# Bazs/structure_from_motion

Measured on NVIDIA B200. Metric: hyp x point evals/sec (fp64), higher is better.
Workload: dtype f64

## Files before the change

### structure_from_motion_b200/csrc/sfm_api.cu

```cuda
#include "../../include/sfm_b200.h"

#include <dlfcn.h>

#include <cmath>
#include <cstdarg>
#include <cstdio>
#include <cstdlib>
#include <cstring>
#include <string>
#include <vector>

#include "sfm_device.cuh"
#include "sfm_fit.cuh"
#include "sfm_linalg.cuh"
#include "sfm_score.cuh"
#include "sfm_homography.cuh"
#include "sfm_pose.cuh"
#include "sfm_tail.cuh"
#include "sfm_misc.cuh"
#include "sfm_match.cuh"
#include "sfm_harris.cuh"
#include "sfm_select.cuh"

using namespace sfm;

static_assert(sizeof(Corr) == 32, "Corr must be 32 bytes");
static_assert(sizeof(PoseSet) == sizeof(sfm_poses), "PoseSet/sfm_poses layout mismatch");
static_assert(sizeof(SelectRecord) == SFM_RECORD_BYTES, "SelectRecord / SFM_RECORD_BYTES mismatch");
static_assert(sizeof(ModelScores) == sizeof(sfm_model_scores), "ModelScores / sfm_model_scores layout mismatch");

namespace {

thread_local std::string g_err;
// ... 43 lines not shown
    T* as() const { return reinterpret_cast<T*>(p); }
    void release() {
        if (p) cudaFree(p);
        p = nullptr;
        cap = 0;
    }
};

enum { T_UPLOAD = 0, T_SAMPLE, T_FIT, T_SCORE, T_SELECT, T_MASK, T_POSE, T_TRI, T_COUNT };

}

struct sfm_ctx {
    int device = 0;
    int sm_count = 148;
    cudaStream_t own_stream = nullptr, stream = nullptr;
    Buf raw, pts, offsets, Ks, table, E, valid, eig;
    Buf acc, count_extra, S1, S2, err, blocks, best, invalid, winnerE, spts, bounds, fitflag, record, merged, rows, blockinv;
    Buf m_img, m_feat, m_W, m_ss, m_ok, m_S, m_out;
    Buf h_img, h_gx, h_gy, h_corner, h_alive, h_key, h_idx, h_small, h_xy;
    Buf mask, sed, poses, pass, X, idx, scan, tmp, tailstate, num, winrec, bout;
    Buf planes, hK;
    Buf selstate, selio, selpp;
    long long n = 0, h = 0, npairs = 1;
    long long first_len = 0;
    long long batch_max_len = 0;
    long long raw_stride = 1;
    bool batched = false, has_pts = false, has_table = false, has_models = false, has_score = false;
    bool models_h = false;
    int hscore_occ = 0;
    bool table_pending = false;
    unsigned long long smp_seed = 0, smp_stream = 0;
    long long smp_offset = 0;
    bool acc_clean = false;
    size_t acc_planes_for = 0;
    double Kstage[9] = {0};
    double hstage[18] = {0};
    std::vector<SelectModels> sstage;
    std::vector<double> Kbatch;
    const void* occ_fn[4] = {nullptr, nullptr, nullptr, nullptr};
    int occ_blocks[4] = {0, 0, 0, 0};
    int occ_next = 0;
    void* nccl_comm = nullptr;
    int nccl_rank = 0, nccl_world = 1;
    Buf gathered;
    const unsigned long long* rescored_dev = nullptr;
    long long winner_local = -1;
    bool winner_set = false;
    long long last_idx_offset = 0;
    double Khost[9] = {1, 0, 0, 0, 1, 0, 0, 0, 1};
    int variant = SFM_SCORE_AUTO, hpt = 2, group = 16;
    bool timing = false;
    cudaEvent_t ev0[T_COUNT], ev1[T_COUNT];
    bool ev_used[T_COUNT];
    long long launches = 0;
    void* hpin = nullptr;
    size_t hpin_cap = 0;

    void tic(int s) {
        if (timing) { cudaEventRecord(ev0[s], stream); }
    }
    void toc(int s) {
        if (timing) { cudaEventRecord(ev1[s], stream); ev_used[s] = true; }
    }
// ... 49 lines not shown
    cfg->attrs = at;
    cfg->numAttrs = SFM_PDL ? 1 : 0;
}
template <typename... KArgs, typename... Args>
cudaError_t chain_launch(sfm_ctx* c, void (*kernel)(KArgs...), dim3 grid, dim3 block, size_t smem, Args&&... args) {
    cudaLaunchConfig_t cfg;
    cudaLaunchAttribute at;
    chain_config(c, grid, block, smem, &cfg, &at);
    return cudaLaunchKernelEx(&cfg, kernel, static_cast<KArgs>(args)...);
}
inline cudaError_t chain_launch_ptr(sfm_ctx* c, const void* fn, dim3 grid, dim3 block, size_t smem, void** kargs) {
    cudaLaunchConfig_t cfg;
    cudaLaunchAttribute at;
    chain_config(c, grid, block, smem, &cfg, &at);
    return cudaLaunchKernelExC(&cfg, fn, kargs);
}

size_t score_warp_smem(int hpt, bool full) {
    switch (hpt) {
        case 1: return full ? score_warp_bytes<1, MODE_FULL>() : sizeof(ScoreWarpSmem<1>);
        case 2: return full ? score_warp_bytes<2, MODE_FULL>() : sizeof(ScoreWarpSmem<2>);
        case 4: return full ? score_warp_bytes<4, MODE_FULL>() : sizeof(ScoreWarpSmem<4>);
        default: return sizeof(ScoreWarpSmem<8>);
    }
}

const void* score_kernel(int variant, int hpt, int group) {
    if (variant == SFM_SCORE_SCREEN32) {
#define SFM_K32(H, G) if (hpt == H && group == G) return reinterpret_cast<const void*>(&k_score<H, G, MODE_SCREEN32>)
        SFM_K32(2, 16); SFM_K32(4, 8); SFM_K32(8, 4);
#undef SFM_K32
        return nullptr;
    }
#define SFM_K(H, G) if (hpt == H && group == G) return scr ? reinterpret_cast<const void*>(&k_score<H, G, MODE_SCREEN>) \
                                                           : reinterpret_cast<const void*>(&k_score<H, G, MODE_FULL>)
    const bool scr = variant == SFM_SCORE_SCREEN;
    SFM_K(1, 16); SFM_K(1, 32);
    SFM_K(2, 4); SFM_K(2, 8); SFM_K(2, 16);
    SFM_K(4, 2); SFM_K(4, 4); SFM_K(4, 8);
#undef SFM_K
    return nullptr;
}

}

extern "C" {
// ... 227 lines not shown
    c->npairs = 1;
    const double* s[4];
    if (on_device) {
        if (int r = c->raw.reserve((size_t)n * 4 * sizeof(double))) return r;
        double* d = c->raw.as<double>();
        const double* src[4] = {xa, ya, xb, yb};
        for (int k = 0; k < 4; ++k) {
            CU(cudaMemcpy2DAsync(d + (size_t)k * n, sizeof(double), src[k], (size_t)stride * sizeof(double),
                                 sizeof(double), (size_t)n, cudaMemcpyDeviceToDevice, c->stream));
            s[k] = d + (size_t)k * n;
        }
        c->raw_stride = stride = 1;
    } else if (int r = stage_raw(c, xa, ya, xb, yb, stride, n, s)) {
        return r;
    }
    if (int r = c->Ks.reserve(9 * sizeof(double))) return r;
    memcpy(c->Khost, K, sizeof c->Khost);
    CU(cudaMemcpyAsync(c->Ks.p, c->Khost, 9 * sizeof(double), cudaMemcpyHostToDevice, c->stream));
    c->n = n;
    if (int r = normalise_from(c, s[0], s[1], s[2], s[3], stride, n, n)) return r;
    c->toc(T_UPLOAD);
    if (sync) CU(cudaStreamSynchronize(c->stream));
    c->has_pts = true;
    c->has_table = c->has_models = c->has_score = false;
    c->table_pending = false;
    c->winner_set = false;
    return 0;
}

int sfm_upload_pairs(sfm_ctx* c, const double* xa, const double* ya, const double* xb, const double* yb,
                     int64_t stride, int64_t n, const double* K) {
    return upload_pairs_impl(c, xa, ya, xb, yb, stride, n, K, false, true);
}

int sfm_upload_pairs_async(sfm_ctx* c, const double* xa, const double* ya, const double* xb, const double* yb,
                           int64_t stride, int64_t n, const double* K) {
    return upload_pairs_impl(c, xa, ya, xb, yb, stride, n, K, false, false);
}

int sfm_upload_pairs_d(sfm_ctx* c, const double* xa, const double* ya, const double* xb, const double* yb,
                       int64_t stride, int64_t n, const double* K) {
    return upload_pairs_impl(c, xa, ya, xb, yb, stride, n, K, true, true);
}

int sfm_get_normalised(sfm_ctx* c, double* out, int64_t n) {
    if (int r = use(c)) return r;
// ... 98 lines not shown
    if (int r = c->S1.reserve(H * 8)) return r;
    if (int r = c->S2.reserve(H * 8)) return r;
    if (int r = c->err.reserve(H * 8)) return r;
    if (int r = c->blocks.reserve((size_t)fblocks * P * sizeof(Best))) return r;
    if (int r = c->best.reserve((size_t)P * sizeof(Best))) return r;
    if (int r = c->invalid.reserve((size_t)P * 16)) return r;
    return 0;
}

struct ItemSplit { long long chunk, nsplit; };
static ItemSplit split_items(long long target_items, long long hyp_items, long long max_len, long long tile) {
    const long long tiles = (max_len + tile - 1) / tile;
    long long nsplit = (target_items + hyp_items - 1) / hyp_items;
    constexpr int min_tiles = 2;
    const long long max_split = tiles / min_tiles > 0 ? tiles / min_tiles : 1;
    if (nsplit > max_split) nsplit = max_split;
    const long long min_split = (max_len + kMaxItemPoints - 1) / kMaxItemPoints;
    if (nsplit < min_split) nsplit = min_split;
    if (nsplit < 1) nsplit = 1;
    const long long chunk = ((tiles + nsplit - 1) / nsplit) * tile;
    nsplit = (max_len + chunk - 1) / chunk;
    if (nsplit < 1) nsplit = 1;
    return {chunk, nsplit};
}

static int clear_acc(sfm_ctx* c, size_t H, long long P) {
    if (!(c->acc_clean && c->acc_planes_for == H))
        CU(cudaMemsetAsync(c->acc.p, 0, H * kAccWords * 8 + acc_tail_bytes(P), c->stream));
    c->acc_clean = false;
    return 0;
}

static int finalise_launch(sfm_ctx* c, int kind, double thr, double min_extra, int agg, int mode, bool use_table,
                           long long idx_offset, int sums, int e2, int force_rescore, unsigned long long* acc_dev) {
    const long long h = c->h, P = c->npairs;
    const size_t H = (size_t)h * P;
    const int fblocks = (int)((h + 255) / 256);
    c->tic(T_SELECT);
    FinalArgs f;
    f.pts = c->pts.as<Corr>();
    f.offsets = c->batched ? c->offsets.as<long long>() : nullptr;
    f.E = c->E.as<double>();
    f.valid = c->valid.as<uint8_t>();
    f.table = use_table ? c->table.as<int32_t>() : nullptr;
    f.h = h;
    f.n = c->n;
// ... 51 lines not shown
    const int G = (c->variant == SFM_SCORE_SCREEN32 && thr > 1e6) ? 16 : c->group;
    const long long hblocks = (h + 32ll * hpt - 1) / (32ll * hpt);
    const size_t H = (size_t)h * P;
    if (int r = reserve_selection(c, h, P)) return r;
    int e2 = 0;
    if (thr > 0.0 && !skip_k2) (void)frexp(thr, &e2);
    if (e2 < -400) e2 = -400;
    const bool autov = c->variant == SFM_SCORE_AUTO;
    int variant = autov ? SFM_SCORE_SCREEN : c->variant;
    if (variant == SFM_SCORE_SCREEN32 && thr > 1e6) variant = SFM_SCORE_SCREEN;
    const bool f32 = variant == SFM_SCORE_SCREEN32;
    const bool screen = variant != SFM_SCORE_FULL;
    double thr_pre = f32 ? thr * kThr32Factor : (screen ? thr * (1.0 + 1e-9) : thr * (1.0 + 1e-9) + 1e-22);
    if (f32 && thr_pre < 1e-24) thr_pre = 1e-24;
    if (screen && thr_pre < 1e-280) thr_pre = 1e-280;
    const double s_scale = sqrt(thr_pre);
    const double scale1 = ldexp(1.0, 63 - e2), scale2 = ldexp(1.0, 63 - 2 * e2);
    unsigned long long* acc_dev = nullptr;
    {
        const void* fn = score_kernel(variant, hpt, G);
        if (!fn) return fail(SFM_ERR_ARG, "unsupported scoring configuration (variant %d, hpt %d, group %d)", variant, hpt, G);
        const size_t smem_one = (size_t)kScoreWarps * score_warp_smem(hpt, false);
        const size_t smem_two = (size_t)kScoreWarps * score_warp_smem(hpt, true);
        const size_t smem_both = smem_one > smem_two ? smem_one : smem_two;
        const size_t smem = screen ? smem_one : smem_two;
        auto occupancy = [&](const void* f, size_t bytes, int* out) -> int {
            for (int k = 0; k < 4; ++k)
                if (c->occ_fn[k] == f) { *out = c->occ_blocks[k]; return 0; }
            int o = 0;
            CU(cudaFuncSetAttribute(f, cudaFuncAttributeMaxDynamicSharedMemorySize, (int)bytes));
            CU(cudaOccupancyMaxActiveBlocksPerMultiprocessor(&o, f, kScoreThreads, bytes));
            if (o < 1) o = 1;
            c->occ_fn[c->occ_next] = f;
            c->occ_blocks[c->occ_next] = o;
            c->occ_next = (c->occ_next + 1) & 3;
            *out = o;
            return 0;
        };
        int occ = 0;
        if (int r = occupancy(fn, smem, &occ)) return r;
#ifndef SFM_AUTO_SINGLE
#define SFM_AUTO_SINGLE 1
#endif
        const void* fn_auto = nullptr;
        if (autov && SFM_AUTO_SINGLE) {
            if (hpt == 2 && G == 16) fn_auto = reinterpret_cast<const void*>(&k_score_auto<2, 16>);
            if (hpt == 4 && G == 8) fn_auto = reinterpret_cast<const void*>(&k_score_auto<4, 8>);
        }
        if (fn_auto)
            if (int r = occupancy(fn_auto, smem_both, &occ)) return r;
        const void* fn_full = (autov && !fn_auto) ? score_kernel(SFM_SCORE_FULL, hpt, G) : nullptr;
        int occ_full = 0;
        if (fn_full)
            if (int r = occupancy(fn_full, smem_two, &occ_full)) return r;
        const long long grid_blocks = (long long)c->sm_count * occ;
        constexpr int items_per_warp = 32;
        const ItemSplit sp = split_items(grid_blocks * kScoreWarps * items_per_warp, hblocks * P, max_len, kTile);
        const long long chunk = sp.chunk, nsplit = sp.nsplit;
        const long long total_items = hblocks * nsplit * P;
        if (int r = c->acc.reserve(H * kAccWords * 8 + acc_tail_bytes(P))) return r;
        const long long npts = c->n;
        if (f32) { if (int r = c->spts.reserve((size_t)npts * sizeof(Corr32))) return r; }
        else if (screen) { if (int r = c->spts.reserve((size_t)npts * sizeof(Corr))) return r; }
        ScoreArgs a;
        a.pts = c->pts.as<Corr>();
        a.spts = screen ? c->spts.p : c->pts.p;
        a.bounds = c->bounds.as<double>();
        a.s = s_scale;
        a.kappa_coef = kKappaCoef * (1.0 + thr);
        a.kappa32_coef = kKappa32Coef * (1.0 + thr);
        a.n = c->n;
        a.offsets = c->batched ? c->offsets.as<long long>() : nullptr;
        a.E = c->E.as<double>();
        a.rows = c->rows.as<ModelRow>();
        a.h = h;
        a.thr = thr;
        a.thr_pre = thr_pre;
        a.scale1 = scale1;
        a.scale2 = scale2;
        a.sums = sums;
        a.chunk = chunk;
        a.hblocks = (int)hblocks;
        a.nsplit = (int)nsplit;
        a.total_items = total_items;
        a.htotal = (long long)H;
        a.acc = c->acc.as<unsigned long long>();
        a.work_counter = reinterpret_cast<unsigned*>(a.acc + H * kAccWords);
        char* tailp = reinterpret_cast<char*>(a.acc + H * kAccWords);
        a.mode_flag = autov ? reinterpret_cast<const int*>(tailp + 32) : nullptr;
        acc_dev = a.acc;
        c->tic(T_SCORE);
        if (int r = clear_acc(c, H, P)) return r;
        if (f32 && !skip_k2) {
            k_screen_pts32<<<(unsigned)((npts + 255) / 256), 256, 0, c->stream>>>(c->pts.as<Corr>(), npts, 1.0 / s_scale,
                                                                                  reinterpret_cast<Corr32*>(c->spts.p));
            if (int r = check_launch(c, "k_screen_pts32")) return r;
        }
        else if (screen && !skip_k2) {
            PilotArgs pa;
            pa.E = c->E.as<double>();
            pa.h = h;
            pa.plen = c->batched ? c->first_len : c->n;
            pa.thr_pre = thr_pre;
            pa.counters = reinterpret_cast<unsigned*>(tailp + 16);
            pa.mode_flag = autov ? reinterpret_cast<int*>(tailp + 32) : nullptr;
            CU(chain_launch(c, k_screen_pts64, dim3((unsigned)((npts + 255) / 256)), dim3(256), 0, c->pts.as<Corr>(), npts,
                            1.0 / s_scale, reinterpret_cast<Corr*>(c->spts.p), pa));
            if (int r = check_launch(c, "k_screen_pts64")) return r;
        }
        const long long want_blocks = (total_items + kScoreWarps - 1) / kScoreWarps;
        const long long launch_blocks = grid_blocks < want_blocks ? grid_blocks : want_blocks;
        void* kargs[] = {(void*)&a};
        if (!skip_k2 && fn_auto) {
            ScoreArgs a2 = a;
            a2.thr_pre = thr * (1.0 + 1e-9) + 1e-22;
            a2.spts = c->pts.p;
            void* kargs2[] = {(void*)&a, (void*)&a2};
            CU(chain_launch_ptr(c, fn_auto, dim3((unsigned)launch_blocks), dim3(kScoreThreads), smem_both, kargs2));
            if (int r = check_launch(c, "k_score_auto")) return r;
        } else if (!skip_k2) {
            CU(chain_launch_ptr(c, fn, dim3((unsigned)launch_blocks), dim3(kScoreThreads), smem, kargs));
            if (int r = check_launch(c, "k_score")) return r;
            if (fn_full) {
                ScoreArgs a2 = a;
                a2.thr_pre = thr * (1.0 + 1e-9) + 1e-22;
                a2.spts = c->pts.p;
                const long long gb2 = (long long)c->sm_count * occ_full;
                const long long lb2 = gb2 < want_blocks ? gb2 : want_blocks;
                void* kargs2[] = {(void*)&a2};
                CU(chain_launch_ptr(c, fn_full, dim3((unsigned)lb2), dim3(kScoreThreads), smem_two, kargs2));
                if (int r = check_launch(c, "k_score")) return r;
            }
        }
        c->toc(T_SCORE);
    }

    return finalise_launch(c, MODEL_E, thr, min_extra, agg, mode, use_table, idx_offset, sums, e2, force_rescore, acc_dev);
}

int sfm_score(sfm_ctx* c, double thr, double min_extra, int agg, int mode, int use_table, int64_t idx_offset,
              int32_t* count_extra, double* S1, double* S2, double* err) {
    if (int r = use(c)) return r;
    if (c->batched) return fail(SFM_ERR_STATE, "sfm_score is a single-pair call; use sfm_batch_ransac");
    if (int r = score_launch(c, thr, min_extra, agg, mode, use_table != 0, idx_offset, c->n, S1 || S2)) return r;
    const size_t H = (size_t)c->h;
    if (count_extra) CU(cudaMemcpyAsync(count_extra, c->count_extra.p, H * 4, cudaMemcpyDeviceToHost, c->stream));
    if (S1) CU(cudaMemcpyAsync(S1, c->S1.p, H * 8, cudaMemcpyDeviceToHost, c->stream));
    if (S2) CU(cudaMemcpyAsync(S2, c->S2.p, H * 8, cudaMemcpyDeviceToHost, c->stream));
// ... 892 lines not shown
    c->npairs = npairs;
    c->n = n;
    c->first_len = offsets[1] - offsets[0];
    if (int r = c->offsets.reserve((size_t)(npairs + 1) * 8)) return r;
    if (int r = c->Ks.reserve((size_t)npairs * 72)) return r;
    CU(cudaMemcpyAsync(c->offsets.p, offsets, (size_t)(npairs + 1) * 8, cudaMemcpyHostToDevice, c->stream));
    CU(cudaMemcpyAsync(c->Ks.p, Ks, (size_t)npairs * 72, cudaMemcpyHostToDevice, c->stream));
    c->Kbatch.assign(Ks, Ks + 9 * npairs);
    c->batch_max_len = max_len;
    const double* s[4];
    if (int r = stage_raw(c, xa, ya, xb, yb, stride, n, s)) return r;
    if (pixels) {
        const double I[9] = {1, 0, 0, 0, 1, 0, 0, 0, 1};
        if (int r = hpose_stage_k(c, I)) return r;
        if (int r = c->pts.reserve((size_t)n * sizeof(Corr))) return r;
        k_normalise<<<dim3((unsigned)((n + 255) / 256), 1), 256, 0, c->stream>>>(s[0], s[1], s[2], s[3], stride, n, nullptr,
                                                                                c->hK.as<double>(), c->pts.as<Corr>(), nullptr);
        if (int r = check_launch(c, "k_normalise")) return r;
    } else if (int r = normalise_from(c, s[0], s[1], s[2], s[3], stride, n, max_len)) {
        return r;
    }
    c->toc(T_UPLOAD);
    c->has_pts = true;
    c->has_table = c->has_models = c->has_score = false;
    c->table_pending = false;
    c->winner_set = false;
    *max_len_out = max_len;
    return 0;
}

static int batch_core(sfm_ctx* c, const double* xa, const double* ya, const double* xb, const double* yb, int64_t stride,
                      const int64_t* offsets, int64_t npairs, const double* Ks, int64_t h, uint64_t seed, uint64_t pair_id0,
                      double thr, double min_extra, int agg, int mode, long long* max_len_out) {
    long long max_len = 0;
    if (int r = batch_upload(c, xa, ya, xb, yb, stride, offsets, npairs, Ks, h, false, &max_len)) return r;
    if (int r = sample_device(c, seed, pair_id0, 0, h)) return r;
    if (int r = fit_launch(c, false)) return r;
    if (int r = score_launch(c, thr, min_extra, agg, mode, true, 0, max_len)) return r;
    *max_len_out = max_len;
    return 0;
}

static int batch_fetch_winners(sfm_ctx* c, int64_t npairs, size_t extra_pinned, char** extra) {
    const size_t rbytes = (size_t)npairs * sizeof(SelectRecord);
    if (int r = ensure_pinned(c, rbytes + extra_pinned + 64)) return r;
    char* hp = (char*)c->hpin;
// ... 403 lines not shown
```

### structure_from_motion_b200/csrc/sfm_score.cuh

```cuda
#pragma once
#include <type_traits>

#include "sfm_device.cuh"

namespace sfm {

__device__ __forceinline__ uint32_t smem_u32(const void* p) {
    return (uint32_t)__cvta_generic_to_shared(p);
}
__device__ __forceinline__ void mbar_init(void* bar, uint32_t count) {
    asm volatile("mbarrier.init.shared::cta.b64 [%0], %1;" ::"r"(smem_u32(bar)), "r"(count) : "memory");
}
__device__ __forceinline__ void mbar_fence_init() {
    asm volatile("fence.mbarrier_init.release.cluster;" ::: "memory");
}
__device__ __forceinline__ void mbar_expect_tx(void* bar, uint32_t bytes) {
    asm volatile("mbarrier.arrive.expect_tx.shared::cta.b64 _, [%0], %1;" ::"r"(smem_u32(bar)), "r"(bytes)
                 : "memory");
}
__device__ __forceinline__ void mbar_wait(void* bar, uint32_t parity) {
    uint32_t ok;
    do {
        asm volatile(
            "{\n\t.reg .pred p;\n\t"
// ... 10 lines not shown
            smem_u32(dst_smem)),
        "l"(src_gmem), "r"(bytes), "r"(smem_u32(bar))
        : "memory");
}

constexpr int kScoreThreads = 128;
constexpr int kScoreWarps = kScoreThreads / 32;
#ifndef SFM_SCORE_TILE
#define SFM_SCORE_TILE 64
#endif
#ifndef SFM_SCORE_STAGES
#define SFM_SCORE_STAGES 3
#endif
constexpr int kTile = SFM_SCORE_TILE;
constexpr int kStages = SFM_SCORE_STAGES;
constexpr int kRing = 64;
constexpr unsigned kMaxPoints = 1u << 25;
constexpr int kChunks = 4;
constexpr int kFixedBits = 21 * kChunks;
constexpr int kChunkBits = 21;
constexpr int kAccWords = 1 + 2 * kChunks;
constexpr long long kMaxItemPoints = 1ll << 11;
enum { SUM_S1 = 1, SUM_S2 = 2 };
enum { MODE_FULL = 0, MODE_SCREEN = 1, MODE_SCREEN32 = 2 };
constexpr double kKappaCoef = 4e-20;
constexpr double kKappa32Coef = 1.2e-10;
constexpr double kThr32Factor = 1.0316;

__global__ void __launch_bounds__(256) k_pad_models(const double* __restrict__ E, long long htotal, ModelRow* __restrict__ rows) {
    const long long i = blockIdx.x * (long long)blockDim.x + threadIdx.x;
    if (i >= htotal) return;
    const double* e = E + 9 * i;
    ModelRow r;
    r.a = make_double4(e[0], e[1], e[2], e[3]);
    r.b = make_double4(e[4], e[5], e[6], e[7]);
    r.c = make_double4(e[8], 0.0, 0.0, 0.0);
    rows[i] = r;
}

struct ScoreArgs {
    const Corr* pts;
    const void* spts;
    const double* bounds;
    long long n;
    const long long* offsets;
    const double* E;
    const ModelRow* rows;
    long long h;
    double thr, thr_pre, s;
    double kappa_coef;
    double kappa32_coef;
    double scale1, scale2;
    int sums;
    long long chunk;
    int hblocks, nsplit;
    long long total_items;
    long long htotal;
    unsigned* work_counter;
    unsigned long long* acc;
    const int* mode_flag;
};

__device__ __forceinline__ unsigned atom_add_acq_rel_shared(unsigned* p, unsigned v) {
    unsigned old;
    asm volatile("atom.acq_rel.cta.shared::cta.add.u32 %0, [%1], %2;" : "=r"(old) : "r"(smem_u32(p)), "r"(v) : "memory");
// ... 8 lines not shown
    unsigned m;
    asm("mov.u32 %0, %%lanemask_lt;" : "=r"(m));
    return m;
}

__device__ __forceinline__ void chunks21(double x, double scale, unsigned (&c)[kChunks]) {
    const double t = x * scale;
    const unsigned long long v = __double2ull_rz(t);
    const double rem = t - __ull2double_rz(v);
    c[0] = (unsigned)__double2uint_rz(rem * 2097152.0);
    c[1] = (unsigned)v & 0x1fffffu;
    c[2] = (unsigned)(v >> kChunkBits) & 0x1fffffu;
    c[3] = (unsigned)(v >> (2 * kChunkBits));
}

struct __align__(16) Corr32 {
    float xa, ya, xb, yb;
};

constexpr int kPilotBlocks = 32;
constexpr int kPilotHyps = 64;
constexpr int kPilotPts = 1024;
constexpr double kPilotFullAbove = 0.09;
struct PilotArgs {
    const double* E;
    long long h;
    long long plen;
    double thr_pre;
    unsigned* counters;
    int* mode_flag;
};
__global__ void __launch_bounds__(256) k_screen_pts64(const Corr* __restrict__ pts, long long n, double inv_s,
                                                      Corr* __restrict__ spts, const PilotArgs pa) {
    chain_enter();
    const long long i = blockIdx.x * (long long)blockDim.x + threadIdx.x;
    if (i < n) {
        Corr c = pts[i];
        c.xa *= inv_s;
        c.ya *= inv_s;
        spts[i] = c;
    }
    if (!pa.mode_flag || blockIdx.x >= kPilotBlocks) return;
    const int nb = gridDim.x < kPilotBlocks ? gridDim.x : kPilotBlocks;
    const long long nh = pa.h < kPilotHyps ? pa.h : kPilotHyps;
    const int hs = threadIdx.x % kPilotHyps;
    int pass = 0, tests = 0;
    if (hs < nh && pa.plen > 0) {
        const long long hyp = (pa.h / nh) * hs;
        double e[9];
#pragma unroll
        for (int k = 0; k < 9; ++k) e[k] = pa.E[9 * hyp + k];
        const long long np = pa.plen < kPilotPts ? pa.plen : kPilotPts;
        const long long step = pa.plen / np;
        const int lanes = nb * (256 / kPilotHyps);
        Corr cs[8];
        int got = 0;
#pragma unroll
        for (int u = 0; u < 8; ++u) {
            const long long q = blockIdx.x * (256 / kPilotHyps) + threadIdx.x / kPilotHyps + (long long)u * lanes;
            if (q < np) { cs[u] = pts[q * step]; got = u + 1; }
        }
#pragma unroll
        for (int u = 0; u < 8; ++u)
            if (u < got) {
                pass += sed_screen(e, cs[u].xa, cs[u].ya, cs[u].xb, cs[u].yb, pa.thr_pre) < 0.0 ? 1 : 0;
                tests += 1;
            }
    }
    unsigned long long v = ((unsigned long long)pass << 32) | (unsigned)tests;
#pragma unroll
    for (int d = 16; d > 0; d >>= 1) v += __shfl_xor_sync(0xffffffffu, v, d);
    __shared__ unsigned long long s_sum;
    __shared__ int s_last;
    if (threadIdx.x == 0) s_sum = 0ull;
    __syncthreads();
    if ((threadIdx.x & 31) == 0) atomicAdd(&s_sum, v);
    __syncthreads();
    if (threadIdx.x == 0) {
        unsigned long long* tot = reinterpret_cast<unsigned long long*>(pa.counters);
        atomicAdd(tot, s_sum);
        __threadfence();
        s_last = atomicAdd(pa.counters + 2, 1u) == (unsigned)(nb - 1);
        if (s_last) {
            __threadfence();
            const unsigned long long t = *reinterpret_cast<volatile unsigned long long*>(tot);
            const double rate = (unsigned)t ? (double)(t >> 32) / (double)(unsigned)t : 0.0;
            *pa.mode_flag = rate > kPilotFullAbove ? MODE_FULL : MODE_SCREEN;
        }
    }
}

__global__ void __launch_bounds__(256) k_screen_pts32(const Corr* __restrict__ pts, long long n, double inv_s,
                                                      Corr32* __restrict__ spts) {
    const long long i = blockIdx.x * (long long)blockDim.x + threadIdx.x;
    if (i >= n) return;
    const Corr c = pts[i];
    Corr32 f;
    f.xa = (float)(c.xa * inv_s); f.ya = (float)(c.ya * inv_s); f.xb = (float)c.xb; f.yb = (float)c.yb;
    spts[i] = f;
}

template <int HPT>
struct alignas(128) ScoreWarpSmem {
    Corr tile[kStages][kTile];
    unsigned sacc[HPT][kAccWords][32];
    uint2 ring[kRing];
    unsigned short own[32];
    unsigned long long full_bar[kStages];
};

constexpr int kTileFS = 32;
constexpr int kStagesFS = 3;
template <int HPT>
struct alignas(128) ScoreWarpSmemFS {
    Corr tile[kStagesFS][kTileFS];
    double model[32 * HPT][10];
    unsigned sacc[HPT][kAccWords][32];
    uint2 ring[kRing];
    unsigned long long full_bar[kStagesFS];
};
__host__ __device__ constexpr bool score_full_in_smem(int hpt) { return hpt <= 2; }
template <int HPT, int MODE>
constexpr size_t score_warp_bytes() {
    return (MODE == MODE_FULL && score_full_in_smem(HPT)) ? sizeof(ScoreWarpSmemFS<HPT>) : sizeof(ScoreWarpSmem<HPT>);
}

#ifndef SFM_SCORE_MINB4
#define SFM_SCORE_MINB4 4
#endif
#ifndef SFM_SCORE_MINB2
#define SFM_SCORE_MINB2 5
#endif
constexpr int score_min_blocks(int hpt) { return hpt >= 4 ? SFM_SCORE_MINB4 : (hpt == 2 ? SFM_SCORE_MINB2 : 8); }


__device__ __forceinline__ int sign_word(double d) { return __double2hiint(d); }
__device__ __forceinline__ int sign_word(float f) { return __float_as_int(f); }

template <int HPT, int G, int MODE>
__device__ __forceinline__ void score_body(const ScoreArgs& a) {
    constexpr bool SCREEN = MODE != MODE_FULL;
    constexpr bool F32 = MODE == MODE_SCREEN32;
    using T = typename std::conditional<F32, float, double>::type;
    using P = typename std::conditional<F32, Corr32, Corr>::type;
    constexpr int NB = HPT * G;
    constexpr bool FS = MODE == MODE_FULL && score_full_in_smem(HPT);
    constexpr bool ENTRY = MODE == MODE_FULL;
    constexpr int TILE = FS ? kTileFS : kTile;
    constexpr int STAGES = FS ? kStagesFS : kStages;
    constexpr int AHEAD = FS ? STAGES - 1 : STAGES;
    using WS = typename std::conditional<FS, ScoreWarpSmemFS<HPT>, ScoreWarpSmem<HPT>>::type;
    static_assert(NB <= 32 && (TILE % G) == 0 && (kTile % TILE) == 0, "a batch is at most 32 tests and divides a tile");
    extern __shared__ __align__(128) unsigned char score_smem[];
    const unsigned full = 0xffffffffu;
    const int lane = threadIdx.x & 31;
    const int warp = __shfl_sync(full, (int)(threadIdx.x >> 5), 0);
    const unsigned lt = lanemask_lt();
    if (a.mode_flag && *a.mode_flag != MODE) return;
    WS& ws = reinterpret_cast<WS*>(score_smem)[warp];

    if (lane == 0) {
#pragma unroll
        for (int s = 0; s < STAGES; ++s) mbar_init(&ws.full_bar[s], 1);
        mbar_fence_init();
    }
#pragma unroll
    for (int j = 0; j < HPT; ++j)
#pragma unroll
        for (int k = 0; k < kAccWords; ++k) ws.sacc[j][k][lane] = 0;
    __syncwarp();
    uint2* q = ws.ring;
    unsigned head = 0, tail = 0;
    unsigned gt = 0;
    const double ab2 = SCREEN ? a.bounds[0] * a.bounds[1] * (F32 ? a.kappa32_coef : a.kappa_coef) : 0.0;

    for (;;) {
        unsigned item = 0;
        if (lane == 0) item = atomicAdd(a.work_counter, 1u);
        item = __shfl_sync(full, item, 0);
        if (item >= a.total_items) break;
        const int hw = (int)(item % (unsigned)a.hblocks);
        const unsigned rest = item / (unsigned)a.hblocks;
        const int split = (int)(rest % (unsigned)a.nsplit);
        const int pair = (int)(rest / (unsigned)a.nsplit);

        const long long pbase = a.offsets ? a.offsets[pair] : 0;
        const long long plen = a.offsets ? a.offsets[pair + 1] - pbase : a.n;
        long long begin = (long long)split * a.chunk;
        if (begin > plen) begin = plen;
        const long long end = pbase + ((begin + a.chunk < plen) ? begin + a.chunk : plen);
        begin += pbase;
        const int ntiles = (int)((end - begin + TILE - 1) / TILE);
        const long long hyp_w = (long long)hw * (32 * HPT);
        const double* Ep = a.E + 9 * (long long)pair * a.h;
        const ModelRow* Rw = a.rows + (long long)pair * a.h + hyp_w;
        const Corr* pbeg = a.pts + begin;
        const P* src = reinterpret_cast<const P*>(SCREEN ? a.spts : (const void*)a.pts);

        auto issue = [&](int t) {
            const int s = (int)((gt + (unsigned)t) % STAGES);
            const long long first = begin + (long long)t * TILE;
            const long long rem = end - first;
            const uint32_t bytes = (uint32_t)((rem < TILE ? rem : TILE) * sizeof(P));
            mbar_expect_tx(&ws.full_bar[s], bytes);
            bulk_g2s(&ws.tile[s][0], src + first, bytes, &ws.full_bar[s]);
        };
        if (lane == 0) {
            for (int t = 0; t < AHEAD && t < ntiles; ++t) issue(t);
        }

        T e[HPT][9], kap[HPT];
#pragma unroll
        for (int j = 0; j < HPT; ++j) {
            const long long hyp = hyp_w + 32 * j + lane;
            const bool real = hyp < a.h;
            double v[9], f2 = 0.0;
#pragma unroll
            for (int k = 0; k < 9; ++k) {
                v[k] = real ? Ep[9 * hyp + k] : 0.0;
                f2 = fma(v[k], v[k], f2);
            }
            if constexpr (FS) {
                double2* mp = reinterpret_cast<double2*>(&ws.model[32 * j + lane][0]);
                mp[0] = make_double2(v[0], v[1]);
                mp[1] = make_double2(v[2], v[3]);
                mp[2] = make_double2(v[4], v[5]);
                mp[3] = make_double2(v[6], v[7]);
                ws.model[32 * j + lane][8] = v[8];
// ... 104 lines not shown
            accumulate(act, survivor_sed(act ? (unsigned)(32 * slot + owner) : 0u, rel), slot, owner);
            head += (unsigned)ndone;
            __syncwarp();
        };
        auto push_records = [&](unsigned vote, unsigned pm, unsigned rel0) {
            if (pm) q[(tail + __popc(vote & lt)) & (kRing - 1)] = make_uint2(pm, ((unsigned)lane << 27) | rel0);
            tail += __popc(vote);
            __syncwarp();
            while (tail - head >= 32u) drain_records();
        };
        auto drain = [&]() {
            if constexpr (ENTRY) drain_entries();
            else drain_records();
        };

        unsigned mark = tail;
        for (int t = 0; t < ntiles; ++t) {
            const unsigned gti = gt + (unsigned)t;
            const int s = (int)(gti % STAGES);
            mbar_wait(&ws.full_bar[s], (gti / STAGES) & 1u);
            const long long first = begin + (long long)t * TILE;
            const int np = (int)((end - first < TILE) ? (end - first) : TILE);
            const P* tp = reinterpret_cast<const P*>(&ws.tile[s][0]);
            for (int p = 0; p < np; p += G) {
                unsigned pm = 0;
#pragma unroll
                for (int g = 0; g < G; ++g) {
                    const P c = tp[p + g];
                    T d[HPT];
                    if (SCREEN) {
                        T t0[HPT], t1[HPT], t2[HPT];
#pragma unroll
                        for (int j = 0; j < HPT; ++j) {
                            t0[j] = fma(c.yb, e[j][3], e[j][6]);
                            t1[j] = fma(c.yb, e[j][4], e[j][7]);
                            t2[j] = fma(c.yb, e[j][5], e[j][8]);
                        }
#pragma unroll
                        for (int j = 0; j < HPT; ++j) {
                            t0[j] = fma(c.xb, e[j][0], t0[j]);
                            t1[j] = fma(c.xb, e[j][1], t1[j]);
                            t2[j] = fma(c.xb, e[j][2], t2[j]);
                        }
#pragma unroll
                        for (int j = 0; j < HPT; ++j) t2[j] = fma(c.ya, t1[j], t2[j]);
#pragma unroll
                        for (int j = 0; j < HPT; ++j) t2[j] = fma(c.xa, t0[j], t2[j]);
#pragma unroll
                        for (int j = 0; j < HPT; ++j) t1[j] = fma(t1[j], t1[j], kap[j]);
#pragma unroll
                        for (int j = 0; j < HPT; ++j) t1[j] = fma(t0[j], t0[j], t1[j]);
#pragma unroll
                        for (int j = 0; j < HPT; ++j) d[j] = fma(t2[j], t2[j], -t1[j]);
                    } else if constexpr (!SCREEN) {
#pragma unroll
                        for (int j = 0; j < HPT; ++j) d[j] = sed_full_decision(e[j], c.xa, c.ya, c.xb, c.yb, a.thr_pre);
                    }
#pragma unroll
                    for (int j = 0; j < HPT; ++j) pm = __funnelshift_l((unsigned)sign_word(d[j]), pm, 1);
                }
                const int v = np - p;
                if (v < G) pm &= 0xffffffffu << (NB - v * HPT);
                const unsigned vote = __ballot_sync(full, pm != 0u);
                if (vote) {
                    if constexpr (ENTRY) push_entries(pm, FS ? (unsigned)(s * TILE + p) : (unsigned)(first - begin) + (unsigned)p);
                    else push_records(vote, pm, (unsigned)(first - begin) + (unsigned)p);
                }
            }
            if constexpr (FS) {
                while ((int)(mark - head) > 0) drain();
                mark = tail;
            }
            __syncwarp();
            if (lane == 0 && t + AHEAD < ntiles) issue(t + AHEAD);
        }
        gt += (unsigned)ntiles;
// ... 6 lines not shown
            const unsigned cnt = ws.sacc[j][0][col];
            if (cnt) {
                unsigned long long* dst = a.acc + (long long)pair * a.h + hyp;
                atomicAdd(dst, (unsigned long long)cnt);
                ws.sacc[j][0][col] = 0;
#pragma unroll
                for (int k = 1; k < kAccWords; ++k) {
                    const unsigned v = ws.sacc[j][k][col];
                    if (v) {
                        atomicAdd(dst + (long long)k * a.htotal, (unsigned long long)v);
                        ws.sacc[j][k][col] = 0;
                    }
                }
            }
        }
        __syncwarp();
    }
}

template <int HPT, int G, int MODE>
__global__ void __launch_bounds__(kScoreThreads, score_min_blocks(MODE == MODE_SCREEN32 ? HPT / 2 : HPT))
k_score(const ScoreArgs a) {
    chain_enter();
    score_body<HPT, G, MODE>(a);
}

template <int HPT, int G>
__global__ void __launch_bounds__(kScoreThreads, score_min_blocks(HPT)) k_score_auto(const ScoreArgs a, const ScoreArgs a_full) {
    chain_enter();
    if (*a.mode_flag == MODE_FULL) score_body<HPT, G, MODE_FULL>(a_full);
    else score_body<HPT, G, MODE_SCREEN>(a);
}

enum { AGG_SUM = 0, AGG_SQUARE = 1, AGG_MEAN = 2, AGG_RMS = 3 };
enum { SELECT_MIN_ERROR = 0, SELECT_MAX_INLIERS = 1, SELECT_MSAC = 2 };

struct Best {
    double err;
    long long idx;
    int count;
    int pad;
};

struct SelectRecord {
    Best best;
    long long num_invalid, first_invalid;
    double E[9];
    int32_t sample[8];
};

__device__ __forceinline__ bool better(const Best& x, const Best& y, int mode) {
    if (y.idx < 0) return x.idx >= 0;
    if (x.idx < 0) return false;
// ... 368 lines not shown
```

Measured before the change: 1029 billion.

## Reorder points by Morton code and use per-tile bounding boxes in screening

Adds a one-time Morton-order sort of correspondences per pair (bbox, keys, CUB radix sort, gather) and computes a per-tile bounding box of the second-image coordinates. In a new MODE_SCREEN_BOX path the per-point gradient-norm term of the screening test is replaced by a conservative per-tile bound computed once per tile per hypothesis. This saves several FMAs per hypothesis-point evaluation in the inner loop. The cost is the sort and gather work, extra buffers, an extra bulk copy per tile, and a looser screening bound that may send more candidates to later stages.

```diff
diff --git a/structure_from_motion_b200/csrc/sfm_api.cu b/structure_from_motion_b200/csrc/sfm_api.cu
--- a/structure_from_motion_b200/csrc/sfm_api.cu
+++ b/structure_from_motion_b200/csrc/sfm_api.cu
@@ -9,6 +9,8 @@
 #include <cstring>
 #include <string>
 #include <vector>
+
+#include <cub/device/device_radix_sort.cuh>
 
 #include "sfm_device.cuh"
 #include "sfm_fit.cuh"
@@ -98,12 +100,14 @@
     Buf mask, sed, poses, pass, X, idx, scan, tmp, tailstate, num, winrec, bout;
     Buf planes, hK;
     Buf selstate, selio, selpp;
+    Buf opts, boxes, order;
     long long n = 0, h = 0, npairs = 1;
     long long first_len = 0;
     long long batch_max_len = 0;
     long long raw_stride = 1;
     bool batched = false, has_pts = false, has_table = false, has_models = false, has_score = false;
     bool models_h = false;
+    bool ordered = false;
     int hscore_occ = 0;
     bool table_pending = false;
     unsigned long long smp_seed = 0, smp_stream = 0;
@@ -116,6 +120,7 @@
     std::vector<double> Kbatch;
     const void* occ_fn[4] = {nullptr, nullptr, nullptr, nullptr};
     int occ_blocks[4] = {0, 0, 0, 0};
+    size_t occ_bytes[4] = {0, 0, 0, 0};
     int occ_next = 0;
     void* nccl_comm = nullptr;
     int nccl_rank = 0, nccl_world = 1;
@@ -211,6 +216,14 @@
         case 2: return full ? score_warp_bytes<2, MODE_FULL>() : sizeof(ScoreWarpSmem<2>);
         case 4: return full ? score_warp_bytes<4, MODE_FULL>() : sizeof(ScoreWarpSmem<4>);
         default: return sizeof(ScoreWarpSmem<8>);
+    }
+}
+size_t score_warp_smem_box(int hpt) {
+    switch (hpt) {
+        case 1: return sizeof(ScoreWarpSmem<1, true>);
+        case 2: return sizeof(ScoreWarpSmem<2, true>);
+        case 4: return sizeof(ScoreWarpSmem<4, true>);
+        default: return sizeof(ScoreWarpSmem<8, true>);
     }
 }
 
@@ -484,6 +497,7 @@
     c->toc(T_UPLOAD);
     if (sync) CU(cudaStreamSynchronize(c->stream));
     c->has_pts = true;
+    c->ordered = false;
     c->has_table = c->has_models = c->has_score = false;
     c->table_pending = false;
     c->winner_set = false;
@@ -628,6 +642,47 @@
     nsplit = (max_len + chunk - 1) / chunk;
     if (nsplit < 1) nsplit = 1;
     return {chunk, nsplit};
+}
+
+static int ensure_ordered(sfm_ctx* c) {
+    if (c->ordered) return 0;
+    const long long n = c->n, P = c->npairs;
+    const long long max_len = c->batched ? c->batch_max_len : n;
+    const long long* off = c->batched ? c->offsets.as<long long>() : nullptr;
+    int pbits = 0;
+    while ((1ll << pbits) < P) ++pbits;
+    const int end_bit = kMortonBits + pbits;
+    size_t sort_bytes = 0;
+    CU(cub::DeviceRadixSort::SortPairs(nullptr, sort_bytes, (const unsigned long long*)nullptr, (unsigned long long*)nullptr,
+                                       (const unsigned*)nullptr, (unsigned*)nullptr, n, 0, end_bit, c->stream));
+    const size_t bb = (size_t)P * 16, kb = ((size_t)n * 8 + 255) & ~(size_t)255, ib = ((size_t)n * 4 + 255) & ~(size_t)255;
+    const size_t bb_al = (bb + 255) & ~(size_t)255;
+    if (int r = c->order.reserve(2 * bb_al + 2 * kb + 2 * ib + sort_bytes)) return r;
+    if (int r = c->opts.reserve((size_t)n * sizeof(Corr))) return r;
+    if (int r = c->boxes.reserve((size_t)(n / kTile + P + 1) * sizeof(double4))) return r;
+    char* w = c->order.as<char>();
+    auto* bmin = reinterpret_cast<unsigned long long*>(w);
+    auto* bmax = reinterpret_cast<unsigned long long*>(w + bb_al);
+    auto* k0 = reinterpret_cast<unsigned long long*>(w + 2 * bb_al);
+    auto* k1 = reinterpret_cast<unsigned long long*>(w + 2 * bb_al + kb);
+    auto* i0 = reinterpret_cast<unsigned*>(w + 2 * bb_al + 2 * kb);
+    auto* i1 = reinterpret_cast<unsigned*>(w + 2 * bb_al + 2 * kb + ib);
+    void* tmp = w + 2 * bb_al + 2 * kb + 2 * ib;
+    CU(cudaMemsetAsync(bmin, 0xff, bb, c->stream));
+    CU(cudaMemsetAsync(bmax, 0, bb, c->stream));
+    const dim3 grid((unsigned)((max_len + 255) / 256), (unsigned)P);
+    const Corr* pts = c->pts.as<Corr>();
+    k_order_bbox<<<grid, 256, 0, c->stream>>>(pts, n, off, bmin, bmax);
+    if (int r = check_launch(c, "k_order_bbox")) return r;
+    k_order_keys<<<grid, 256, 0, c->stream>>>(pts, n, off, bmin, bmax, k0, i0);
+    if (int r = check_launch(c, "k_order_keys")) return r;
+    CU(cub::DeviceRadixSort::SortPairs(tmp, sort_bytes, k0, k1, i0, i1, n, 0, end_bit, c->stream));
+    const long long tiles = (max_len + kTile - 1) / kTile;
+    k_order_gather_boxes<<<dim3((unsigned)((tiles + 7) / 8), (unsigned)P), 256, 0, c->stream>>>(
+        pts, n, off, i1, c->opts.as<Corr>(), c->boxes.as<double4>());
+    if (int r = check_launch(c, "k_order_gather_boxes")) return r;
+    c->ordered = true;
+    return 0;
 }
 
 static int clear_acc(sfm_ctx* c, size_t H, long long P) {
@@ -725,23 +780,27 @@
         if (!fn) return fail(SFM_ERR_ARG, "unsupported scoring configuration (variant %d, hpt %d, group %d)", variant, hpt, G);
         const size_t smem_one = (size_t)kScoreWarps * score_warp_smem(hpt, false);
         const size_t smem_two = (size_t)kScoreWarps * score_warp_smem(hpt, true);
-        const size_t smem_both = smem_one > smem_two ? smem_one : smem_two;
-        const size_t smem = screen ? smem_one : smem_two;
-        auto occupancy = [&](const void* f, size_t bytes, int* out) -> int {
+        const size_t smem_box = (size_t)kScoreWarps * score_warp_smem_box(hpt);
+        size_t smem_both = smem_one > smem_two ? smem_one : smem_two;
+        if (smem_box > smem_both) smem_both = smem_box;
+        const bool dense = screen && !f32 && c->n >= kBoxMinPairLen * P;
+        const size_t smem = screen ? (dense && !autov ? smem_box : smem_one) : smem_two;
+        auto occupancy = [&](const void* f, size_t bytes, size_t cap, int* out) -> int {
             for (int k = 0; k < 4; ++k)
-                if (c->occ_fn[k] == f) { *out = c->occ_blocks[k]; return 0; }
+                if (c->occ_fn[k] == f && c->occ_bytes[k] == bytes) { *out = c->occ_blocks[k]; return 0; }
             int o = 0;
-            CU(cudaFuncSetAttribute(f, cudaFuncAttributeMaxDynamicSharedMemorySize, (int)bytes));
+            CU(cudaFuncSetAttribute(f, cudaFuncAttributeMaxDynamicSharedMemorySize, (int)(cap > bytes ? cap : bytes)));
             CU(cudaOccupancyMaxActiveBlocksPerMultiprocessor(&o, f, kScoreThreads, bytes));
             if (o < 1) o = 1;
             c->occ_fn[c->occ_next] = f;
+            c->occ_bytes[c->occ_next] = bytes;
             c->occ_blocks[c->occ_next] = o;
             c->occ_next = (c->occ_next + 1) & 3;
             *out = o;
             return 0;
         };
         int occ = 0;
-        if (int r = occupancy(fn, smem, &occ)) return r;
+        if (int r = occupancy(fn, smem, (screen && !f32) ? smem_box : smem, &occ)) return r;
 #ifndef SFM_AUTO_SINGLE
 #define SFM_AUTO_SINGLE 1
 #endif
@@ -751,11 +810,11 @@
             if (hpt == 4 && G == 8) fn_auto = reinterpret_cast<const void*>(&k_score_auto<4, 8>);
         }
         if (fn_auto)
-            if (int r = occupancy(fn_auto, smem_both, &occ)) return r;
+            if (int r = occupancy(fn_auto, smem_both, smem_both, &occ)) return r;
         const void* fn_full = (autov && !fn_auto) ? score_kernel(SFM_SCORE_FULL, hpt, G) : nullptr;
         int occ_full = 0;
         if (fn_full)
-            if (int r = occupancy(fn_full, smem_two, &occ_full)) return r;
+            if (int r = occupancy(fn_full, smem_two, smem_two, &occ_full)) return r;
         const long long grid_blocks = (long long)c->sm_count * occ;
         constexpr int items_per_warp = 32;
         const ItemSplit sp = split_items(grid_blocks * kScoreWarps * items_per_warp, hblocks * P, max_len, kTile);
@@ -763,11 +822,15 @@
         const long long total_items = hblocks * nsplit * P;
         if (int r = c->acc.reserve(H * kAccWords * 8 + acc_tail_bytes(P))) return r;
         const long long npts = c->n;
+        const bool boxed = dense && (!autov || fn_auto);
         if (f32) { if (int r = c->spts.reserve((size_t)npts * sizeof(Corr32))) return r; }
-        else if (screen) { if (int r = c->spts.reserve((size_t)npts * sizeof(Corr))) return r; }
+        else if (screen) { if (int r = c->spts.reserve((size_t)npts * sizeof(Corr) * (boxed ? 2 : 1))) return r; }
+        if (boxed && !skip_k2)
+            if (int r = ensure_ordered(c)) return r;
         ScoreArgs a;
         a.pts = c->pts.as<Corr>();
         a.spts = screen ? c->spts.p : c->pts.p;
+        a.boxes = nullptr;
         a.bounds = c->bounds.as<double>();
         a.s = s_scale;
         a.kappa_coef = kKappaCoef * (1.0 + thr);
@@ -791,6 +854,12 @@
         a.work_counter = reinterpret_cast<unsigned*>(a.acc + H * kAccWords);
         char* tailp = reinterpret_cast<char*>(a.acc + H * kAccWords);
         a.mode_flag = autov ? reinterpret_cast<const int*>(tailp + 32) : nullptr;
+        ScoreArgs a_box = a;
+        if (boxed) {
+            a_box.pts = c->opts.as<Corr>();
+            a_box.spts = c->spts.as<Corr>() + npts;
+            a_box.boxes = c->boxes.as<double4>();
+        }
         acc_dev = a.acc;
         c->tic(T_SCORE);
         if (int r = clear_acc(c, H, P)) return r;
@@ -807,18 +876,20 @@
             pa.thr_pre = thr_pre;
             pa.counters = reinterpret_cast<unsigned*>(tailp + 16);
             pa.mode_flag = autov ? reinterpret_cast<int*>(tailp + 32) : nullptr;
-            CU(chain_launch(c, k_screen_pts64, dim3((unsigned)((npts + 255) / 256)), dim3(256), 0, c->pts.as<Corr>(), npts,
-                            1.0 / s_scale, reinterpret_cast<Corr*>(c->spts.p), pa));
+            pa.box_ok = boxed ? 1 : 0;
+            CU(chain_launch(c, k_screen_pts64, dim3((unsigned)((npts + 255) / 256)), dim3(256), 0, c->pts.as<Corr>(),
+                            boxed ? c->opts.as<Corr>() : nullptr, npts, 1.0 / s_scale, reinterpret_cast<Corr*>(c->spts.p), pa));
             if (int r = check_launch(c, "k_screen_pts64")) return r;
         }
         const long long want_blocks = (total_items + kScoreWarps - 1) / kScoreWarps;
         const long long launch_blocks = grid_blocks < want_blocks ? grid_blocks : want_blocks;
-        void* kargs[] = {(void*)&a};
+        void* kargs[] = {boxed ? (void*)&a_box : (void*)&a};
         if (!skip_k2 && fn_auto) {
             ScoreArgs a2 = a;
             a2.thr_pre = thr * (1.0 + 1e-9) + 1e-22;
+            a2.pts = c->pts.as<Corr>();
             a2.spts = c->pts.p;
-            void* kargs2[] = {(void*)&a, (void*)&a2};
+            void* kargs2[] = {(void*)&a, (void*)&a_box, (void*)&a2};
             CU(chain_launch_ptr(c, fn_auto, dim3((unsigned)launch_blocks), dim3(kScoreThreads), smem_both, kargs2));
             if (int r = check_launch(c, "k_score_auto")) return r;
         } else if (!skip_k2) {
@@ -827,6 +898,7 @@
             if (fn_full) {
                 ScoreArgs a2 = a;
                 a2.thr_pre = thr * (1.0 + 1e-9) + 1e-22;
+                a2.pts = c->pts.as<Corr>();
                 a2.spts = c->pts.p;
                 const long long gb2 = (long long)c->sm_count * occ_full;
                 const long long lb2 = gb2 < want_blocks ? gb2 : want_blocks;
@@ -1765,6 +1837,7 @@
     }
     c->toc(T_UPLOAD);
     c->has_pts = true;
+    c->ordered = false;
     c->has_table = c->has_models = c->has_score = false;
     c->table_pending = false;
     c->winner_set = false;
diff --git a/structure_from_motion_b200/csrc/sfm_score.cuh b/structure_from_motion_b200/csrc/sfm_score.cuh
--- a/structure_from_motion_b200/csrc/sfm_score.cuh
+++ b/structure_from_motion_b200/csrc/sfm_score.cuh
@@ -56,10 +56,13 @@
 constexpr int kAccWords = 1 + 2 * kChunks;
 constexpr long long kMaxItemPoints = 1ll << 11;
 enum { SUM_S1 = 1, SUM_S2 = 2 };
-enum { MODE_FULL = 0, MODE_SCREEN = 1, MODE_SCREEN32 = 2 };
+enum { MODE_FULL = 0, MODE_SCREEN = 1, MODE_SCREEN32 = 2, MODE_SCREEN_BOX = 3 };
 constexpr double kKappaCoef = 4e-20;
 constexpr double kKappa32Coef = 1.2e-10;
 constexpr double kThr32Factor = 1.0316;
+constexpr double kBoxRound = 1e-15;
+constexpr double kBoxGrow = 1.0 + 4e-15;
+constexpr long long kBoxMinPairLen = 32768;
 
 __global__ void __launch_bounds__(256) k_pad_models(const double* __restrict__ E, long long htotal, ModelRow* __restrict__ rows) {
     const long long i = blockIdx.x * (long long)blockDim.x + threadIdx.x;
@@ -75,6 +78,7 @@
 struct ScoreArgs {
     const Corr* pts;
     const void* spts;
+    const double4* boxes;
     const double* bounds;
     long long n;
     const long long* offsets;
@@ -129,6 +133,7 @@
 constexpr int kPilotHyps = 64;
 constexpr int kPilotPts = 1024;
 constexpr double kPilotFullAbove = 0.09;
+constexpr double kPilotBoxBelow = 0.02;
 struct PilotArgs {
     const double* E;
     long long h;
@@ -136,9 +141,10 @@
     double thr_pre;
     unsigned* counters;
     int* mode_flag;
+    int box_ok;
 };
-__global__ void __launch_bounds__(256) k_screen_pts64(const Corr* __restrict__ pts, long long n, double inv_s,
-                                                      Corr* __restrict__ spts, const PilotArgs pa) {
+__global__ void __launch_bounds__(256) k_screen_pts64(const Corr* __restrict__ pts, const Corr* __restrict__ opts, long long n,
+                                                      double inv_s, Corr* __restrict__ spts, const PilotArgs pa) {
     chain_enter();
     const long long i = blockIdx.x * (long long)blockDim.x + threadIdx.x;
     if (i < n) {
@@ -146,6 +152,12 @@
         c.xa *= inv_s;
         c.ya *= inv_s;
         spts[i] = c;
+        if (opts) {
+            c = opts[i];
+            c.xa *= inv_s;
+            c.ya *= inv_s;
+            spts[n + i] = c;
+        }
     }
     if (!pa.mode_flag || blockIdx.x >= kPilotBlocks) return;
     const int nb = gridDim.x < kPilotBlocks ? gridDim.x : kPilotBlocks;
@@ -192,7 +204,8 @@
             __threadfence();
             const unsigned long long t = *reinterpret_cast<volatile unsigned long long*>(tot);
             const double rate = (unsigned)t ? (double)(t >> 32) / (double)(unsigned)t : 0.0;
-            *pa.mode_flag = rate > kPilotFullAbove ? MODE_FULL : MODE_SCREEN;
+            *pa.mode_flag = rate > kPilotFullAbove ? MODE_FULL
+                            : ((pa.box_ok && rate < kPilotBoxBelow) ? MODE_SCREEN_BOX : MODE_SCREEN);
         }
     }
 }
@@ -207,13 +220,120 @@
     spts[i] = f;
 }
 
-template <int HPT>
+constexpr int kMortonBits = 20;
+__device__ __forceinline__ unsigned long long ord_bits(double x) {
+    const unsigned long long b = (unsigned long long)__double_as_longlong(x);
+    return (b >> 63) ? ~b : (b | 0x8000000000000000ull);
+}
+__device__ __forceinline__ double ord_value(unsigned long long o) {
+    return __longlong_as_double((long long)((o >> 63) ? (o & 0x7fffffffffffffffull) : ~o));
+}
+__device__ __forceinline__ unsigned spread10(unsigned v) {
+    v &= 0x3ffu;
+    v = (v | (v << 8)) & 0x00ff00ffu;
+    v = (v | (v << 4)) & 0x0f0f0f0fu;
+    v = (v | (v << 2)) & 0x33333333u;
+    return (v | (v << 1)) & 0x55555555u;
+}
+__host__ __device__ __forceinline__ long long tile_box_index(long long base, long long pair, long long k) {
+    return base / kTile + pair + k;
+}
+__device__ __forceinline__ unsigned long long shfl_xor_u64(unsigned long long v, int d) {
+    return __shfl_xor_sync(0xffffffffu, v, d);
+}
+
+__global__ void __launch_bounds__(256) k_order_bbox(const Corr* __restrict__ pts, long long n, const long long* __restrict__ offsets,
+                                                    unsigned long long* __restrict__ bmin, unsigned long long* __restrict__ bmax) {
+    const int p = blockIdx.y;
+    const long long base = offsets ? offsets[p] : 0, len = offsets ? offsets[p + 1] - base : n;
+    const long long i = blockIdx.x * (long long)blockDim.x + threadIdx.x;
+    unsigned long long lo[2] = {~0ull, ~0ull}, hi[2] = {0ull, 0ull};
+    if (i < len) {
+        const Corr c = pts[base + i];
+        const double v[2] = {c.xb, c.yb};
+#pragma unroll
+        for (int k = 0; k < 2; ++k)
+            if (isfinite(v[k])) lo[k] = hi[k] = ord_bits(v[k]);
+    }
+#pragma unroll
+    for (int k = 0; k < 2; ++k) {
+#pragma unroll
+        for (int d = 16; d > 0; d >>= 1) {
+            const unsigned long long l = shfl_xor_u64(lo[k], d), h = shfl_xor_u64(hi[k], d);
+            lo[k] = l < lo[k] ? l : lo[k];
+            hi[k] = h > hi[k] ? h : hi[k];
+        }
+        if ((threadIdx.x & 31) == 0 && hi[k]) {
+            atomicMin(bmin + 2 * p + k, lo[k]);
+            atomicMax(bmax + 2 * p + k, hi[k]);
+        }
+    }
+}
+
+__global__ void __launch_bounds__(256) k_order_keys(const Corr* __restrict__ pts, long long n, const long long* __restrict__ offsets,
+                                                    const unsigned long long* __restrict__ bmin,
+                                                    const unsigned long long* __restrict__ bmax,
+                                                    unsigned long long* __restrict__ keys, unsigned* __restrict__ idx) {
+    const int p = blockIdx.y;
+    const long long base = offsets ? offsets[p] : 0, len = offsets ? offsets[p + 1] - base : n;
+    const long long i = blockIdx.x * (long long)blockDim.x + threadIdx.x;
+    if (i >= len) return;
+    const Corr c = pts[base + i];
+    unsigned g[2];
+    const double v[2] = {c.xb, c.yb};
+#pragma unroll
+    for (int k = 0; k < 2; ++k) {
+        const double lo = ord_value(bmin[2 * p + k]), hi = ord_value(bmax[2 * p + k]);
+        const double sc = hi > lo ? 1023.0 / (hi - lo) : 0.0;
+        g[k] = (unsigned)fmin(fmax((v[k] - lo) * sc, 0.0), 1023.0);
+    }
+    keys[base + i] = ((unsigned long long)p << kMortonBits) | (spread10(g[0]) | (spread10(g[1]) << 1));
+    idx[base + i] = (unsigned)(base + i);
+}
+
+__global__ void __launch_bounds__(256) k_order_gather_boxes(const Corr* __restrict__ pts, long long n,
+                                                            const long long* __restrict__ offsets,
+                                                            const unsigned* __restrict__ idx, Corr* __restrict__ opts,
+                                                            double4* __restrict__ boxes) {
+    const int p = blockIdx.y;
+    const long long base = offsets ? offsets[p] : 0, len = offsets ? offsets[p + 1] - base : n;
+    const long long k = blockIdx.x * (256ll / 32) + (threadIdx.x >> 5);
+    const int lane = threadIdx.x & 31;
+    if (k * kTile >= len) return;
+    const double inf = __longlong_as_double(0x7ff0000000000000LL);
+    double lo[2] = {inf, inf}, hi[2] = {-inf, -inf};
+#pragma unroll
+    for (int r = lane; r < kTile; r += 32) {
+        const long long q = k * kTile + r;
+        if (q < len) {
+            const Corr c = pts[idx[base + q]];
+            opts[base + q] = c;
+            lo[0] = fmin(lo[0], c.xb); hi[0] = fmax(hi[0], c.xb);
+            lo[1] = fmin(lo[1], c.yb); hi[1] = fmax(hi[1], c.yb);
+        }
+    }
+    double ctr[2], half[2];
+#pragma unroll
+    for (int a = 0; a < 2; ++a) {
+#pragma unroll
+        for (int d = 16; d > 0; d >>= 1) {
+            lo[a] = fmin(lo[a], __shfl_xor_sync(0xffffffffu, lo[a], d));
+            hi[a] = fmax(hi[a], __shfl_xor_sync(0xffffffffu, hi[a], d));
+        }
+        ctr[a] = 0.5 * lo[a] + 0.5 * hi[a];
+        half[a] = fmax(__dsub_ru(hi[a], ctr[a]), __dsub_ru(ctr[a], lo[a]));
+    }
+    if (lane == 0) boxes[tile_box_index(base, p, k)] = make_double4(ctr[0], ctr[1], half[0], half[1]);
+}
+
+template <int HPT, bool BOX = false>
 struct alignas(128) ScoreWarpSmem {
     Corr tile[kStages][kTile];
     unsigned sacc[HPT][kAccWords][32];
     uint2 ring[kRing];
     unsigned short own[32];
     unsigned long long full_bar[kStages];
+    double4 box[BOX ? kStages : 1];
 };
 
 constexpr int kTileFS = 32;
@@ -253,11 +373,13 @@
     constexpr int NB = HPT * G;
     constexpr bool FS = MODE == MODE_FULL && score_full_in_smem(HPT);
     constexpr bool ENTRY = MODE == MODE_FULL;
+    constexpr bool BOX = MODE == MODE_SCREEN_BOX;
     constexpr int TILE = FS ? kTileFS : kTile;
     constexpr int STAGES = FS ? kStagesFS : kStages;
     constexpr int AHEAD = FS ? STAGES - 1 : STAGES;
-    using WS = typename std::conditional<FS, ScoreWarpSmemFS<HPT>, ScoreWarpSmem<HPT>>::type;
+    using WS = typename std::conditional<FS, ScoreWarpSmemFS<HPT>, ScoreWarpSmem<HPT, BOX>>::type;
     static_assert(NB <= 32 && (TILE % G) == 0 && (kTile % TILE) == 0, "a batch is at most 32 tests and divides a tile");
+    static_assert(!BOX || TILE == kTile, "a box covers one kTile-record tile");
     extern __shared__ __align__(128) unsigned char score_smem[];
     const unsigned full = 0xffffffffu;
     const int lane = threadIdx.x & 31;
@@ -304,13 +426,15 @@
         const Corr* pbeg = a.pts + begin;
         const P* src = reinterpret_cast<const P*>(SCREEN ? a.spts : (const void*)a.pts);
 
+        const double4* bx = BOX ? a.boxes + tile_box_index(pbase, pair, (begin - pbase) / TILE) : nullptr;
         auto issue = [&](int t) {
             const int s = (int)((gt + (unsigned)t) % STAGES);
             const long long first = begin + (long long)t * TILE;
             const long long rem = end - first;
             const uint32_t bytes = (uint32_t)((rem < TILE ? rem : TILE) * sizeof(P));
-            mbar_expect_tx(&ws.full_bar[s], bytes);
+            mbar_expect_tx(&ws.full_bar[s], bytes + (BOX ? (uint32_t)sizeof(double4) : 0u));
             bulk_g2s(&ws.tile[s][0], src + first, bytes, &ws.full_bar[s]);
+            if constexpr (BOX) bulk_g2s(&ws.box[s], bx + t, (uint32_t)sizeof(double4), &ws.full_bar[s]);
         };
         if (lane == 0) {
             for (int t = 0; t < AHEAD && t < ntiles; ++t) issue(t);
@@ -461,6 +585,23 @@
             const long long first = begin + (long long)t * TILE;
             const int np = (int)((end - first < TILE) ? (end - first) : TILE);
             const P* tp = reinterpret_cast<const P*>(&ws.tile[s][0]);
+            T mb[HPT];
+            if constexpr (BOX) {
+                const double4 b = ws.box[s];
+                const double ax = fabs(b.x) + b.z, ay = fabs(b.y) + b.w;
+#pragma unroll
+                for (int j = 0; j < HPT; ++j) {
+                    double bk[2];
+#pragma unroll
+                    for (int k = 0; k < 2; ++k) {
+                        const double u = e[j][k], v = e[j][3 + k], w = e[j][6 + k];
+                        const double ctr = fma(b.x, u, fma(b.y, v, w));
+                        const double big = fma(fabs(u), ax, fma(fabs(v), ay, fabs(w)));
+                        bk[k] = fma(kBoxRound, big, fma(fabs(u), b.z, fma(fabs(v), b.w, fabs(ctr))));
+                    }
+                    mb[j] = fmin(fma(bk[0], bk[0], fma(bk[1], bk[1], kap[j])) * kBoxGrow, __longlong_as_double(0x7ff0000000000000LL));
+                }
+            }
             for (int p = 0; p < np; p += G) {
                 unsigned pm = 0;
 #pragma unroll
@@ -485,12 +626,17 @@
                         for (int j = 0; j < HPT; ++j) t2[j] = fma(c.ya, t1[j], t2[j]);
 #pragma unroll
                         for (int j = 0; j < HPT; ++j) t2[j] = fma(c.xa, t0[j], t2[j]);
-#pragma unroll
-                        for (int j = 0; j < HPT; ++j) t1[j] = fma(t1[j], t1[j], kap[j]);
-#pragma unroll
-                        for (int j = 0; j < HPT; ++j) t1[j] = fma(t0[j], t0[j], t1[j]);
-#pragma unroll
-                        for (int j = 0; j < HPT; ++j) d[j] = fma(t2[j], t2[j], -t1[j]);
+                        if constexpr (BOX) {
+#pragma unroll
+                            for (int j = 0; j < HPT; ++j) d[j] = fma(t2[j], t2[j], -mb[j]);
+                        } else {
+#pragma unroll
+                            for (int j = 0; j < HPT; ++j) t1[j] = fma(t1[j], t1[j], kap[j]);
+#pragma unroll
+                            for (int j = 0; j < HPT; ++j) t1[j] = fma(t0[j], t0[j], t1[j]);
+#pragma unroll
+                            for (int j = 0; j < HPT; ++j) d[j] = fma(t2[j], t2[j], -t1[j]);
+                        }
                     } else if constexpr (!SCREEN) {
 #pragma unroll
                         for (int j = 0; j < HPT; ++j) d[j] = sed_full_decision(e[j], c.xa, c.ya, c.xb, c.yb, a.thr_pre);
@@ -543,13 +689,19 @@
 __global__ void __launch_bounds__(kScoreThreads, score_min_blocks(MODE == MODE_SCREEN32 ? HPT / 2 : HPT))
 k_score(const ScoreArgs a) {
     chain_enter();
-    score_body<HPT, G, MODE>(a);
+    if constexpr (MODE == MODE_SCREEN) {
+        if (a.boxes) score_body<HPT, G, MODE_SCREEN_BOX>(a);
+        else score_body<HPT, G, MODE_SCREEN>(a);
+    } else {
+        score_body<HPT, G, MODE>(a);
+    }
 }
 
 template <int HPT, int G>
-__global__ void __launch_bounds__(kScoreThreads, score_min_blocks(HPT)) k_score_auto(const ScoreArgs a, const ScoreArgs a_full) {
+__global__ void __launch_bounds__(kScoreThreads, score_min_blocks(HPT)) k_score_auto(const ScoreArgs a, const ScoreArgs a_box, const ScoreArgs a_full) {
     chain_enter();
     if (*a.mode_flag == MODE_FULL) score_body<HPT, G, MODE_FULL>(a_full);
+    else if (*a.mode_flag == MODE_SCREEN_BOX) score_body<HPT, G, MODE_SCREEN_BOX>(a_box);
     else score_body<HPT, G, MODE_SCREEN>(a);
 }
 
```

New measurement: 1056 billion, median of 6. +2.7%, better.
